# yusuke1127/RoboManipBaselines

Measured on AMD Instinct MI355X. Metric: env-steps/s (whole node) + policy-inference us/step, MujocoUR5eCable x N ACT, higher is better.
Workload: dtype f64 physics + fp32 policy; 1 GPU; MujocoUR5eCable x1024 (1024 per GPU), ACT (ResNet-18 + transformer 4/7 layers, chunk 100, skip 3, temporal ensembling), fp32 policy, RolloutPhase hot loop; num_envs_per_gpu=1024, total_envs=1024, parallelism=single GPU (no collective), env_groups=1, act_decoder_layers_run=1

## Files before the change

include/rmbx.h:

```cpp
#ifndef RMBX_H_
#define RMBX_H_

#include <stddef.h>
#include <stdint.h>

#ifdef __cplusplus
extern "C" {
#endif

#define RMBX_OK 0
#define RMBX_ERR_ARG -1
#define RMBX_ERR_HIP -2
#define RMBX_ERR_STATE -3

#define RMBX_ABI_VERSION 2

int rmbx_abi_version(void);
const char* rmbx_last_error(void);
int rmbx_device_count(int* count);

int rmbx_act_ensemble(const float* new_chunk, const uint8_t* push, const uint8_t* active,
                      float* hist, int32_t* hist_len, int32_t* hist_head,
                      const double* w_table, const double* dn_scale, const double* dn_sub,
                      const double* dn_add, double* out, int n_env, int chunk, int adim,
// ... 228 lines not shown
int rmbx_conv3x3_f16x3_patch(const float* in, int N, int H, int W, int C, const void* w_planes,
                             long long w_plane_stride, const float* w_scale, const float* bias, const float* res,
                             float* out, int Cout, int relu, void* stream);
int rmbx_conv2d_f16x3(const float* in, int N, int H, int W, int C, const void* w_planes, const float* w_scale,
                      const float* bias, const float* res, float* out, int Cout, int KH, int KW, int stride, int pad,
                      int relu, void* stream);
int rmbx_attention_f32x6(const float* q, const float* k, const float* v, float* out, int B, int heads, int Lq, int Lk,
                         long long q_bstride, int q_rstride, long long k_bstride, int k_rstride, long long v_bstride,
                         int v_rstride, float scale, void* stream);
int rmbx_attention_f16x3(const float* q, const float* k, const float* v, float* out, int* redo, int B, int heads,
                         int Lq, int Lk, long long q_bstride, int q_rstride, long long k_bstride, int k_rstride,
                         long long v_bstride, int v_rstride, float scale, void* stream);
int rmbx_groupnorm_act(const float* x, const float* weight, const float* bias, float* out, int B, int C, int T,
                       int groups, float eps, int mish, void* stream);
int rmbx_add_layernorm(const void* x, const void* r, const float* weight, const float* bias, void* out,
                       int rows, int D, float eps, int dtype, void* stream);
int rmbx_add_layernorm_pos(const void* x, const void* r, const float* weight, const float* bias, void* out,
                           const void* pos, int pos_rows, void* out_pos, int rows, int D, float eps, int dtype,
                           void* stream);
int rmbx_add_layernorm_split(const float* x, const float* r, const float* weight, const float* bias, float* out,
                             void* y_planes, float* y_rinv, float* y_norm, const float* pos, int pos_rows,
                             float* out_pos, void* pos_planes, float* pos_rinv, int rows, int D, float eps,
                             void* stream);
int rmbx_nhwc_bias_relu_maxpool(const void* x, const float* bias, void* out, int N, int H, int W,
                                int C, int dtype, void* stream);

int rmbx_ddpm_step(const float* model_output, const float* sample, const float* noise,
                   float* prev_sample, size_t n, const float* coeffs, void* stream);
int rmbx_ddim_step(const float* model_output, const float* sample, float* prev_sample, size_t n,
                   const float* coeffs, int eps_mode, void* stream);

int rmbx_resize_crop_u8(const uint8_t* src, int n_env, int H, int W, int C, int rh, int rw, int y0,
                        int x0, int ch, int cw, float a, float b, void* dst, int dst_dtype,
                        void* stream);
int rmbx_resize_f32(const float* src, float* dst, int n_env, int H, int W, int rh, int rw,
                    void* stream);

int rmbx_pointcloud_fps(const float* depth, const uint8_t* rgb, int n_env, int H, int W,
                        double focal_scaling, const double* min_bound, const double* max_bound,
                        int K, int norm_type, const double* norm_a, const double* norm_b,
                        const double* norm_c, float* out, double* raw, int32_t* count,
                        void* stream);

#ifdef __cplusplus
}
#endif
// ... 3 lines not shown
```

robomanipbaselines_amd/_native.py:

```python

import ctypes
import os

import numpy as np

_LIB_PATH = os.path.join(os.path.dirname(os.path.abspath(__file__)), "_lib",
                         f"librmbx_{os.environ['RMBX_LIB_VARIANT']}.so" if os.environ.get("RMBX_LIB_VARIANT")
                         else "librmbx.so")

_c_int = ctypes.c_int
_c_p = ctypes.c_void_p
_c_sz = ctypes.c_size_t
_c_d = ctypes.c_double

SIGNATURES = {
    "rmbx_abi_version": (_c_int, []),
    "rmbx_last_error": (ctypes.c_char_p, []),
    "rmbx_device_count": (_c_int, [_c_p]),
    "rmbx_act_ensemble": (
        _c_int,
        [_c_p] * 11 + [_c_int, _c_int, _c_int, _c_int, _c_p],
    ),
    "rmbx_cable_reward": (_c_int, [_c_p] * 5 + [_c_int, _c_int, _c_p]),
    "rmbx_door_reward": (_c_int, [_c_p, _c_p, _c_p, _c_p, _c_int, _c_d, _c_d, _c_p]),
# ... 42 lines not shown
    "rmbx_attention_f16x3": (_c_int, [_c_p] * 5 + [_c_int] * 4 + [ctypes.c_longlong, _c_int] * 3 + [ctypes.c_float, _c_p]),
    "rmbx_linear_f32x6": (_c_int, [_c_p, ctypes.c_longlong, _c_p, ctypes.c_longlong, ctypes.c_longlong, _c_p, _c_p,
                                   ctypes.c_longlong, _c_int, _c_int, _c_int, _c_int, _c_p]),
    "rmbx_conv2d_f32x6": (_c_int, [_c_p] + [_c_int] * 4 + [_c_p] * 4 + [_c_int] * 6 + [_c_p]),
    "rmbx_linear_f32x6_batched": (_c_int, [_c_p, ctypes.c_longlong, ctypes.c_longlong, _c_p, ctypes.c_longlong,
                                           ctypes.c_longlong, ctypes.c_longlong, _c_p, _c_p, ctypes.c_longlong,
                                           ctypes.c_longlong] + [_c_int] * 5 + [_c_p]),
    "rmbx_wino4_input_f32": (_c_int, [_c_p] + [_c_int] * 4 + [_c_p, _c_p]),
    "rmbx_wino4_output_f32": (_c_int, [_c_p] + [_c_int] * 4 + [_c_p] * 3 + [_c_int, _c_p]),
    "rmbx_conv2d_direct_f32": (_c_int, [_c_p] + [_c_int] * 4 + [_c_p] * 3 + [_c_int] * 5 + [_c_p]),
    "rmbx_split_bf16x3": (_c_int, [_c_p, _c_p, ctypes.c_longlong, _c_p]),
    "rmbx_split_f16x2": (_c_int, [_c_p, _c_int, _c_int, _c_p, _c_p, _c_p]),
    "rmbx_linear_f16x3": (_c_int, [_c_p, ctypes.c_longlong, _c_p, ctypes.c_longlong, ctypes.c_longlong, _c_p, _c_p,
                                   _c_p, ctypes.c_longlong, _c_int, _c_int, _c_int, _c_int, _c_p]),
    "rmbx_linear_f16x3_batched": (_c_int, [_c_p, ctypes.c_longlong, ctypes.c_longlong, _c_p, ctypes.c_longlong,
                                           ctypes.c_longlong, ctypes.c_longlong, _c_p, ctypes.c_longlong, _c_p, _c_p,
                                           ctypes.c_longlong, ctypes.c_longlong] + [_c_int] * 5 + [_c_p]),
    "rmbx_conv3x3_f16x3_patch": (_c_int, [_c_p] + [_c_int] * 4 + [_c_p, ctypes.c_longlong] + [_c_p] * 4
                                 + [_c_int, _c_int, _c_p]),
    "rmbx_conv2d_f16x3": (_c_int, [_c_p] + [_c_int] * 4 + [_c_p] * 5 + [_c_int] * 6 + [_c_p]),
    "rmbx_add_layernorm": (_c_int, [_c_p] * 5 + [_c_int, _c_int, ctypes.c_float, _c_int, _c_p]),
    "rmbx_groupnorm_act": (_c_int, [_c_p] * 4 + [_c_int] * 4 + [ctypes.c_float, _c_int, _c_p]),
    "rmbx_add_layernorm_split": (_c_int, [_c_p] * 9 + [_c_int, _c_p, _c_p, _c_p, _c_int, _c_int, ctypes.c_float, _c_p]),
    "rmbx_linear_f16x3_presplit_split": (_c_int, [_c_p, ctypes.c_longlong, ctypes.c_longlong, _c_p, _c_p, _c_p,
                                                  ctypes.c_longlong, ctypes.c_longlong, _c_p, ctypes.c_float,
                                                  ctypes.c_float, _c_p, _c_int, _c_p, ctypes.c_longlong,
                                                  ctypes.c_longlong, _c_p, _c_int, _c_int, _c_int, _c_p]),
    "rmbx_linear_f16x3_presplit_batched": (_c_int, [_c_p, ctypes.c_longlong, ctypes.c_longlong, ctypes.c_longlong, _c_p,
                                                    ctypes.c_longlong, _c_p, ctypes.c_longlong, ctypes.c_longlong,
                                                    ctypes.c_longlong, _c_p, ctypes.c_longlong, _c_p, _c_p,
                                                    ctypes.c_longlong, ctypes.c_longlong, _c_int, _c_int, _c_int, _c_int,
                                                    _c_int, _c_p]),
    "rmbx_wino4_input_split": (_c_int, [_c_p, _c_int, _c_int, _c_int, _c_int, _c_p, _c_p, _c_p]),
    "rmbx_linear_f16x3_presplit": (_c_int, [_c_p, ctypes.c_longlong, ctypes.c_longlong, _c_p, _c_p, ctypes.c_longlong,
                                            ctypes.c_longlong, _c_p, _c_p, _c_p, _c_p, ctypes.c_longlong, _c_int, _c_int,
                                            _c_int, _c_int, _c_p]),
    "rmbx_add_layernorm_pos": (_c_int, [_c_p] * 6 + [_c_int, _c_p, _c_int, _c_int, ctypes.c_float, _c_int, _c_p]),
    "rmbx_ddpm_step": (_c_int, [_c_p] * 4 + [_c_sz, _c_p, _c_p]),
    "rmbx_ddim_step": (_c_int, [_c_p] * 3 + [_c_sz, _c_p, _c_int, _c_p]),
    "rmbx_resize_crop_u8": (_c_int, [_c_p] + [_c_int] * 10 + [ctypes.c_float, ctypes.c_float, _c_p, _c_int, _c_p]),
    "rmbx_resize_f32": (_c_int, [_c_p, _c_p] + [_c_int] * 5 + [_c_p]),
    "rmbx_pointcloud_fps": (_c_int, [_c_p, _c_p, _c_int, _c_int, _c_int, _c_d, _c_p, _c_p, _c_int, _c_int,
                                     _c_p, _c_p, _c_p, _c_p, _c_p, _c_p, _c_p]),
}


# ... 99 lines not shown
```

robomanipbaselines_amd/csrc/rmbx_nn.hip:

```cpp

#include "rmbx_common.h"

#include <cstdint>
#include <type_traits>

namespace rmbx {
namespace {

__device__ __forceinline__ float bf2f(uint16_t h) { return __uint_as_float((uint32_t)h << 16); }

__device__ __forceinline__ uint16_t f2bf(float f) {
  uint32_t u = __float_as_uint(f);
  if ((u & 0x7fffffffu) > 0x7f800000u) return 0x7fc0;
  u += 0x7fffu + ((u >> 16) & 1u);
  return (uint16_t)(u >> 16);
}

struct BF16 {
  static constexpr int VEC = 8;
  using vec_t = uint4;
  __device__ static void unpack(const vec_t& v, float* f) {
    const uint32_t w[4] = {v.x, v.y, v.z, v.w};
#pragma unroll
    for (int i = 0; i < 4; ++i) {
// ... 164 lines not shown
  const int g = rmbx::grid_for((size_t)N * Ho * Wo * cvec);
  if (dtype == 1)
    hipLaunchKernelGGL(rmbx::bias_relu_maxpool_kernel<rmbx::BF16>, dim3(g), dim3(256), 0, s,
                       (const uint4*)x, bias, (uint4*)out, N, H, W, cvec, Ho, Wo);
  else
    hipLaunchKernelGGL(rmbx::bias_relu_maxpool_kernel<rmbx::F32>, dim3(g), dim3(256), 0, s,
                       (const float4*)x, bias, (float4*)out, N, H, W, cvec, Ho, Wo);
  RMBX_CHECK_LAUNCH();
  return RMBX_OK;
}

namespace rmbx {
namespace {

struct LnSplit {
  uint16_t* y_planes;
  float* y_rinv;
  uint16_t* pos_planes;
  float* pos_rinv;
  int rows;
  float* y_norm;
};

template <class T, int PER>
__global__ void __launch_bounds__(256) add_layernorm_kernel(const typename T::vec_t* __restrict__ x,
                                                            const typename T::vec_t* __restrict__ r,
                                                            const float* __restrict__ w, const float* __restrict__ b,
                                                            typename T::vec_t* __restrict__ out, int rows, int D,
                                                            float eps, const typename T::vec_t* __restrict__ pos,
                                                            int pos_rows, typename T::vec_t* __restrict__ out_pos,
                                                            LnSplit sp) {
  constexpr int V = T::VEC;
  const int lane = threadIdx.x & 63;
  const int row = blockIdx.x * 4 + (threadIdx.x >> 6);
  if (row >= rows) return;
  const int nvec = D / V;
  const size_t base = (size_t)row * nvec;
  float s[PER][V], s2[PER][V];
  float sum = 0.f;
#pragma unroll
  for (int q = 0; q < PER; ++q) {
    const int v = lane + q * 64;
    if (v < nvec) {
      float a[V], c[V];
      T::unpack(x[base + v], a);
      if (r) {
        T::unpack(r[base + v], c);
#pragma unroll
        for (int k = 0; k < V; ++k) a[k] = T::round(a[k] + c[k]);
      }
#pragma unroll
      for (int k = 0; k < V; ++k) {
        s[q][k] = a[k];
        sum += a[k];
      }
    } else {
#pragma unroll
      for (int k = 0; k < V; ++k) s[q][k] = 0.f;
    }
  }
#pragma unroll
  for (int off = 32; off > 0; off >>= 1) sum += __shfl_xor(sum, off);
  const float mean = sum / (float)D;
  float var = 0.f;
#pragma unroll
  for (int q = 0; q < PER; ++q) {
    const int v = lane + q * 64;
    if (v < nvec) {
#pragma unroll
      for (int k = 0; k < V; ++k) {
// ... 34 lines not shown
#pragma unroll
        for (int k = 0; k < V; ++k) yr[k] = yr[k] + pv[k];
        const typename T::vec_t pvv = T::pack(yr);
        if (out_pos) out_pos[base + v] = pvv;
        if (sp.pos_planes) {
          T::unpack(pvv, yr);
#pragma unroll
          for (int k = 0; k < V; ++k) pmax = fmaxf(pmax, fabsf(yr[k]));
        }
      }
      {
        float t[V];
        T::unpack(yv, t);
#pragma unroll
        for (int k = 0; k < V; ++k) s[q][k] = t[k];
      }
      if (sp.pos_planes) {
#pragma unroll
        for (int k = 0; k < V; ++k) s2[q][k] = yr[k];
      }
    }
  }
  if constexpr (std::is_same<T, F32>::value) {
    auto split_row = [&](float (*vals)[V], float mx, uint16_t* planes, float* rinv) {
#pragma unroll
      for (int off = 32; off > 0; off >>= 1) mx = fmaxf(mx, __shfl_xor(mx, off));
      int e = 14;
      if (mx > 0.f && mx <= 3.4e38f) frexpf(mx, &e);
      const float sc = ldexpf(1.f, 14 - e);
      if (lane == 0) rinv[row] = ldexpf(1.f, e - 14);
      const size_t plane = (size_t)sp.rows * D;
#pragma unroll
      for (int q = 0; q < PER; ++q) {
        const int v = lane + q * 64;
        if (v < nvec) {
          uint16_t h[V], l[V];
#pragma unroll
          for (int k = 0; k < V; ++k) {
            const float a = vals[q][k] * sc;
            const _Float16 hv = (_Float16)a;
            h[k] = __builtin_bit_cast(uint16_t, hv);
            l[k] = __builtin_bit_cast(uint16_t, (_Float16)(a - (float)hv));
          }
          static_assert(V == 4, "f32 rows move as float4");
          const size_t o = (size_t)row * D + (size_t)v * V;
          *(uint2*)(planes + o) = make_uint2(h[0] | ((uint32_t)h[1] << 16), h[2] | ((uint32_t)h[3] << 16));
          *(uint2*)(planes + plane + o) = make_uint2(l[0] | ((uint32_t)l[1] << 16), l[2] | ((uint32_t)l[3] << 16));
        }
      }
    };
    if (sp.y_norm) {
      float q = ysq;
#pragma unroll
      for (int off = 32; off > 0; off >>= 1) q += __shfl_xor(q, off);
      if (lane == 0) sp.y_norm[row] = sqrtf(q) * (1.f + 0.000244140625f);
    }
    if (sp.y_planes) split_row(s, ymax, sp.y_planes, sp.y_rinv);
    if (sp.pos_planes) split_row(s2, pmax, sp.pos_planes, sp.pos_rinv);
  }
}

}
}

extern "C" int rmbx_add_layernorm_pos(const void* x, const void* r, const float* weight, const float* bias, void* out,
                                      const void* pos, int pos_rows, void* out_pos, int rows, int D, float eps,
                                      int dtype, void* stream);

extern "C" int rmbx_add_layernorm(const void* x, const void* r, const float* weight, const float* bias, void* out,
                                  int rows, int D, float eps, int dtype, void* stream) {
  return rmbx_add_layernorm_pos(x, r, weight, bias, out, nullptr, 0, nullptr, rows, D, eps, dtype, stream);
}

namespace {
int add_layernorm_impl(const void* x, const void* r, const float* weight, const float* bias, void* out,
                       const void* pos, int pos_rows, void* out_pos, int rows, int D, float eps, int dtype,
                       void* stream, rmbx::LnSplit sp) {
  RMBX_CHECK_ARG(!(out_pos || sp.pos_planes) || (pos && pos_rows > 0),
                 "rmbx_add_layernorm_pos: out_pos needs pos and pos_rows > 0");
  RMBX_CHECK_ARG(((uintptr_t)pos | (uintptr_t)out_pos) % 16 == 0, "rmbx_add_layernorm_pos: unaligned");
  RMBX_CHECK_ARG(x && weight && bias && (out || sp.y_planes || sp.pos_planes), "rmbx_add_layernorm: null pointer");
  RMBX_CHECK_ARG(dtype == 0 || dtype == 1, "rmbx_add_layernorm: dtype must be 0 (f32) or 1 (bf16)");
  const int vec = dtype == 1 ? 8 : 4;
  RMBX_CHECK_ARG(D > 0 && D % vec == 0 && D <= 2048, "rmbx_add_layernorm: D=%d must be a multiple of %d, <= 2048",
                 D, vec);
  RMBX_CHECK_ARG(((uintptr_t)x | (uintptr_t)r | (uintptr_t)out) % 16 == 0, "rmbx_add_layernorm: unaligned");
  if (rows <= 0) return RMBX_OK;
  hipStream_t s = (hipStream_t)stream;
  const int grid = (rows + 3) / 4;
  const int nvec = D / vec;
  if (dtype == 1) {
    if (nvec <= 64)
      hipLaunchKernelGGL((rmbx::add_layernorm_kernel<rmbx::BF16, 1>), dim3(grid), dim3(256), 0, s, (const uint4*)x,
                         (const uint4*)r, weight, bias, (uint4*)out, rows, D, eps, (const uint4*)pos, pos_rows,
                         (uint4*)out_pos, sp);
    else if (nvec <= 128)
      hipLaunchKernelGGL((rmbx::add_layernorm_kernel<rmbx::BF16, 2>), dim3(grid), dim3(256), 0, s, (const uint4*)x,
                         (const uint4*)r, weight, bias, (uint4*)out, rows, D, eps, (const uint4*)pos, pos_rows,
                         (uint4*)out_pos, sp);
    else
      hipLaunchKernelGGL((rmbx::add_layernorm_kernel<rmbx::BF16, 4>), dim3(grid), dim3(256), 0, s, (const uint4*)x,
                         (const uint4*)r, weight, bias, (uint4*)out, rows, D, eps, (const uint4*)pos, pos_rows,
                         (uint4*)out_pos, sp);
  } else {
    if (nvec <= 64)
      hipLaunchKernelGGL((rmbx::add_layernorm_kernel<rmbx::F32, 1>), dim3(grid), dim3(256), 0, s, (const float4*)x,
                         (const float4*)r, weight, bias, (float4*)out, rows, D, eps, (const float4*)pos, pos_rows,
                         (float4*)out_pos, sp);
    else if (nvec <= 128)
      hipLaunchKernelGGL((rmbx::add_layernorm_kernel<rmbx::F32, 2>), dim3(grid), dim3(256), 0, s, (const float4*)x,
                         (const float4*)r, weight, bias, (float4*)out, rows, D, eps, (const float4*)pos, pos_rows,
                         (float4*)out_pos, sp);
    else if (nvec <= 256)
      hipLaunchKernelGGL((rmbx::add_layernorm_kernel<rmbx::F32, 4>), dim3(grid), dim3(256), 0, s, (const float4*)x,
                         (const float4*)r, weight, bias, (float4*)out, rows, D, eps, (const float4*)pos, pos_rows,
                         (float4*)out_pos, sp);
    else
      hipLaunchKernelGGL((rmbx::add_layernorm_kernel<rmbx::F32, 8>), dim3(grid), dim3(256), 0, s, (const float4*)x,
                         (const float4*)r, weight, bias, (float4*)out, rows, D, eps, (const float4*)pos, pos_rows,
                         (float4*)out_pos, sp);
  }
  RMBX_CHECK_LAUNCH();
  return RMBX_OK;
}
}

extern "C" int rmbx_add_layernorm_pos(const void* x, const void* r, const float* weight, const float* bias, void* out,
                                      const void* pos, int pos_rows, void* out_pos, int rows, int D, float eps,
                                      int dtype, void* stream) {
  return add_layernorm_impl(x, r, weight, bias, out, pos, pos_rows, out_pos, rows, D, eps, dtype, stream,
                            rmbx::LnSplit{nullptr, nullptr, nullptr, nullptr, rows, nullptr});
}

extern "C" int rmbx_add_layernorm_split(const float* x, const float* r, const float* weight, const float* bias,
                                        float* out, void* y_planes, float* y_rinv, float* y_norm, const float* pos,
                                        int pos_rows, float* out_pos, void* pos_planes, float* pos_rinv, int rows, int D,
                                        float eps, void* stream) {
  RMBX_CHECK_ARG(!y_planes == !y_rinv && !pos_planes == !pos_rinv, "rmbx_add_layernorm_split: planes need their rinv");
  RMBX_CHECK_ARG(D % 4 == 0 && ((uintptr_t)y_planes | (uintptr_t)pos_planes) % 8 == 0,
                 "rmbx_add_layernorm_split: D %% 4 and 8-byte aligned planes");
  return add_layernorm_impl(x, r, weight, bias, out, pos, pos_rows, out_pos, rows, D, eps, 0, stream,
                            rmbx::LnSplit{(uint16_t*)y_planes, y_rinv, (uint16_t*)pos_planes, pos_rinv, rows, y_norm});
}

namespace rmbx {
namespace {

__device__ __forceinline__ float gn_block_sum(float v, float* red) {
#pragma unroll
  for (int o = 32; o > 0; o >>= 1) v += __shfl_xor(v, o);
  const int wave = threadIdx.x >> 6;
  __syncthreads();
  if ((threadIdx.x & 63) == 0) red[wave] = v;
  __syncthreads();
  return red[0] + red[1] + red[2] + red[3];
}

constexpr int GN_REG = 8;
template <bool MISH, bool TIN>
__global__ void __launch_bounds__(256) groupnorm_act_kernel(const float* __restrict__ x, const float* __restrict__ w,
                                                            const float* __restrict__ b, float* __restrict__ y, int C,
                                                            int T, int G, float eps) {
  __shared__ float red[4];
  const int bg = blockIdx.x, g = bg % G, cg = C / G;
  const int E = cg * T, tid = threadIdx.x;
// ... 93 lines not shown
```

robomanipbaselines_amd/kernels.py:

```python

import os
import numpy as np
import torch

from . import _native as N


def _chk(t, dtype, shape=None, name="tensor"):
    if not isinstance(t, torch.Tensor):
        raise ValueError(f"{name} must be a torch.Tensor")
    if not t.is_cuda:
        raise ValueError(f"{name} must be a device tensor (got {t.device})")
    if t.dtype != dtype:
        raise ValueError(f"{name} must be {dtype} (got {t.dtype})")
    if not t.is_contiguous():
        raise ValueError(f"{name} must be contiguous")
    if shape is not None and tuple(t.shape) != tuple(shape):
        raise ValueError(f"{name} must have shape {tuple(shape)} (got {tuple(t.shape)})")
    return t


def ensemble_weight_table(chunk, k=0.01):
    w = np.zeros((chunk, chunk), dtype=np.float64)
    for n in range(1, chunk + 1):
# ... 477 lines not shown
                      torch.empty(rows, dtype=torch.float32, device=x.device) if y_norm else None) if split_y else None
    yp = ps = pos2 = None
    if pos is not None:
        pos2 = pos.reshape(-1, D)
        if pos2.dtype != x.dtype or not pos2.is_contiguous() or not pos2.is_cuda:
            raise ValueError("pos must be a contiguous device tensor of x's dtype")
        if x.dim() < 2 or x.shape[-2] % pos2.shape[0] != 0:
            raise ValueError("pos rows must divide the sequence length")
        yp = torch.empty_like(x)
        if split_pos:
            ps = PresplitRows(torch.empty((2, rows, D), dtype=torch.float16, device=x.device),
                              torch.empty(rows, dtype=torch.float32, device=x.device))
    N.call("rmbx_add_layernorm_split", N.ptr(x), N.ptr(r), N.ptr(weight), N.ptr(bias), N.ptr(y),
           N.ptr(ys.planes if ys else None), N.ptr(ys.rinv if ys else None), N.ptr(ys.norm if ys else None), N.ptr(pos2),
           pos2.shape[0] if pos2 is not None else 0, N.ptr(yp), N.ptr(ps.planes if ps else None),
           N.ptr(ps.rinv if ps else None), rows, D, float(eps), N.stream_ptr())
    if ys is not None:
        ys.bind(y)
        y.rmbx_split = ys
    if ps is not None:
        ps.bind(yp)
        yp.rmbx_split = ps
    return (y, yp) if pos is not None else y


def weight_bounds(w, b):
    wn = float(w.detach().double().norm(dim=1).max()) if w.numel() else 0.0
    bm = float(b.detach().double().abs().max()) if b is not None and b.numel() else 0.0
    up = 1.0 + 2.0 ** -20
    return wn * up, bm * up


def linear_presplit_split(xs, planes, bias, bounds, relu=False, out=None):
    Nn, K, h3 = _planes_nk(planes, "linear_presplit_split")
    if not h3 or xs.norm is None or xs.planes.shape[2] != K:
        raise ValueError("linear_presplit_split: f16x3 planes and pre-split rows with norm bounds of width K")
    M = xs.planes.shape[1]
    if bias is not None:
        _chk(bias, torch.float32, (Nn,), "bias")
    if out is None:
        out = PresplitRows(torch.empty((2, M, Nn), dtype=torch.float16, device=xs.planes.device),
                           torch.empty(M, dtype=torch.float32, device=xs.planes.device))
    elif (tuple(out.planes.shape) != (2, M, Nn) or out.planes.dtype != torch.float16 or out.planes.stride(2) != 1
          or tuple(out.rinv.shape) != (M,) or out.rinv.dtype != torch.float32 or not out.rinv.is_contiguous()):
        raise ValueError("linear_presplit_split: out must hold [2, M, N] f16 planes (unit column stride) and [M] f32 rinv")
    p, ap, op = planes.planes, xs.planes, out.planes
# ... 606 lines not shown
```

robomanipbaselines_amd/policy/act/act_model.py:

```python

import math
import os

import torch
import torch.nn as nn
import torch.nn.functional as F

from ..backbone import FusedResNet18Trunk, ResNet18Trunk

IMAGENET_MEAN = (0.485, 0.456, 0.406)
IMAGENET_STD = (0.229, 0.224, 0.225)


def sine_pos_embed(h, w, num_pos_feats=256, temperature=10000, device=None, dtype=torch.float32):
    scale = 2 * math.pi
    eps = 1e-6
    ones = torch.ones(1, h, w, device=device, dtype=torch.float32)
    y_embed = ones.cumsum(1)
    x_embed = ones.cumsum(2)
    y_embed = y_embed / (y_embed[:, -1:, :] + eps) * scale
    x_embed = x_embed / (x_embed[:, :, -1:] + eps) * scale
    dim_t = torch.arange(num_pos_feats, dtype=torch.float32, device=device)
    dim_t = temperature ** (2 * (dim_t // 2) / num_pos_feats)
    pos_x = x_embed[:, :, :, None] / dim_t
# ... 81 lines not shown
    def _out_proj(self, o):
        if self.fused_attention and _x6_ok(o, self.out_proj.out_features):
            return _x6_linear(self, "out_proj", o, self.out_proj.weight, self.out_proj.bias)
        return self.out_proj(o)

    def forward(self, q, k, v):
        D = q.shape[2]
        if q is k and k is v:
            qkv = self._in_proj(q, 0, 3 * D)
            qq, kk, vv = qkv.split(D, dim=-1)
        elif q is k:
            qk = self._in_proj(q, 0, 2 * D)
            qq, kk = qk.split(D, dim=-1)
            vv = self._in_proj(v, 2 * D, 3 * D)
        else:
            qq = self._in_proj(q, 0, D)
            kk = self._in_proj(k, D, 2 * D)
            vv = self._in_proj(v, 2 * D, 3 * D)
        return self._attend(qq, kk, vv)

    def attend_kv(self, q, kk, vv):
        D = q.shape[2]
        return self._attend(self._in_proj(q, 0, D), kk, vv)

    def _attend(self, qq, kk, vv):
        B, Lq, D = qq.shape
        Lk = kk.shape[1]
        hd = D // self.h
        if self.fused_attention and qq.dtype == torch.bfloat16 and hd == 64 and Lk <= 320 and qq.is_cuda:
            from ... import kernels as K

            return self._out_proj(K.attention_bf16(qq, kk, vv, self.h))
        if self.fused_attention and qq.dtype == torch.float32 and hd == 64 and qq.is_cuda:
            from ... import kernels as K

            return self._out_proj(K.attention_f32(qq, kk, vv, self.h, form=F32_ATTN))
        qq = qq.view(B, Lq, self.h, hd).transpose(1, 2)
        kk = kk.view(B, Lk, self.h, hd).transpose(1, 2)
        vv = vv.view(B, Lk, self.h, hd).transpose(1, 2)
        o = F.scaled_dot_product_attention(qq, kk, vv)
        return self.out_proj(o.transpose(1, 2).reshape(B, Lq, D))


class _LayerOps(nn.Module):

    fused = False
# ... 28 lines not shown
        cache = norm.__dict__.get("_f32")
        if cache is None or cache[0] != key:
            cache = (key, norm.weight.detach().float().contiguous(), norm.bias.detach().float().contiguous())
            norm.__dict__["_f32"] = cache
        return cache[1], cache[2]

    @staticmethod
    def _presplit(x):
        from ... import kernels as K

        return (x.dtype == torch.float32 and F32_GEMM == "x6" and K.F32_PIECES == "f16x3" and K.GEMM_PRESPLIT
                and x.is_cuda and x.shape[-1] % K.LINEAR_F32X6_BK == 0)

    def addnorm(self, norm, x, r):
        if self.fused:
            from ... import kernels as K

            w, b = self._norm_f32(norm)
            if self._presplit(x):
                return K.add_layernorm_split(x.contiguous(), r.contiguous(), w, b, norm.eps, y_norm=True)
            return K.add_layernorm(x.contiguous(), r.contiguous(), w, b, norm.eps)
        return norm(x + r)

    def addnorm_pos(self, norm, x, r, pos):
        if self.fused:
            from ... import kernels as K

            w, b = self._norm_f32(norm)
            if self._presplit(x):
                return K.add_layernorm_split(x.contiguous(), r.contiguous(), w, b, norm.eps, pos=pos.contiguous(),
                                             split_y=False)
            return K.add_layernorm_pos(x.contiguous(), r.contiguous(), w, b, pos.contiguous(), norm.eps)
        y = norm(x + r)
        return y, y + pos


class EncoderLayer(_LayerOps):
    def __init__(self, d, heads, ff):
        super().__init__()
        self.self_attn = MHA(d, heads)
        self.linear1, self.linear2 = nn.Linear(d, ff), nn.Linear(ff, d)
        self.norm1, self.norm2 = nn.LayerNorm(d), nn.LayerNorm(d)

    def forward(self, src, pos):
        q = src + pos
        src = self.addnorm(self.norm1, src, self.self_attn(q, q, src))
        return self.addnorm(self.norm2, src, self.ffn(src))

    def forward_q(self, src, q, pos, want_next_q):
        src = self.addnorm(self.norm1, src, self.self_attn(q, q, src))
        if want_next_q:
            return self.addnorm_pos(self.norm2, src, self.ffn(src), pos)
        return self.addnorm(self.norm2, src, self.ffn(src)), None


class DecoderLayer(_LayerOps):
    def __init__(self, d, heads, ff):
        super().__init__()
        self.self_attn = MHA(d, heads)
        self.multihead_attn = MHA(d, heads)
        self.linear1, self.linear2 = nn.Linear(d, ff), nn.Linear(ff, d)
        self.norm1, self.norm2, self.norm3 = nn.LayerNorm(d), nn.LayerNorm(d), nn.LayerNorm(d)

    def forward(self, tgt, memory, pos, query_pos, mem_pos=None):
        q = tgt + query_pos
        tgt = self.addnorm(self.norm1, tgt, self.self_attn(q, q, tgt))
        mk = memory + pos if mem_pos is None else mem_pos
        tgt = self.addnorm(self.norm2, tgt, self.multihead_attn(tgt + query_pos, mk, memory))
        return self.addnorm(self.norm3, tgt, self.ffn(tgt))

    def forward_q(self, tgt, q, memory, query_pos, mem_pos, want_next_q, cross_kv=None):
        tgt, q2 = self.addnorm_pos(self.norm1, tgt, self.self_attn(q, q, tgt), query_pos)
        if cross_kv is not None:
            ca = self.multihead_attn.attend_kv(q2, *cross_kv)
        else:
            ca = self.multihead_attn(q2, mem_pos, memory)
        tgt = self.addnorm(self.norm2, tgt, ca)
        if want_next_q:
            return self.addnorm_pos(self.norm3, tgt, self.ffn(tgt), query_pos)
        return self.addnorm(self.norm3, tgt, self.ffn(tgt)), None


class ActModel(nn.Module):

    def __init__(self, state_dim=7, action_dim=7, num_queries=100, hidden_dim=512, dim_feedforward=3200,
                 nheads=8, enc_layers=4, dec_layers=7, num_cams=1, latent_dim=32):
        super().__init__()
        d = hidden_dim
        self.num_queries, self.num_cams, self.latent_dim = num_queries, num_cams, latent_dim
        self.backbone = ResNet18Trunk()
        self.input_proj = nn.Conv2d(512, d, kernel_size=1)
        self.input_proj_robot_state = nn.Linear(state_dim, d)
        self.latent_out_proj = nn.Linear(latent_dim, d)
        self.query_embed = nn.Embedding(num_queries, d)
        self.additional_pos_embed = nn.Embedding(2, d)
        self.encoder_layers = nn.ModuleList([EncoderLayer(d, nheads, dim_feedforward) for _ in range(enc_layers)])
        self.decoder_layers = nn.ModuleList([DecoderLayer(d, nheads, dim_feedforward) for _ in range(dec_layers)])
        self.decoder_norm = nn.LayerNorm(d)
        self.action_head = nn.Linear(d, action_dim)
        self.is_pad_head = nn.Linear(d, 1)
# ... 20 lines not shown
        layers = self.decoder_layers[:n_dec]
        if not self.batch_cross_kv or n_dec < 2 or not all(getattr(l, "fused", False) for l in layers):
            return None
        D = mem.shape[2]
        ws = [l.multihead_attn.in_proj_weight for l in layers]
        bs = [l.multihead_attn.in_proj_bias for l in layers]
        key = tuple((w.data_ptr(), w.dtype) for w in ws)
        cache = self.__dict__.get("_cross_w")
        if cache is None or cache[0] != key:
            wk = torch.cat([w[D: 2 * D] for w in ws]).contiguous()
            bk = torch.cat([b[D: 2 * D] for b in bs]).contiguous()
            wv = torch.cat([w[2 * D:] for w in ws]).contiguous()
            bv = torch.cat([b[2 * D:] for b in bs]).contiguous()
            cache = (key, wk, bk, wv, bv)
            self.__dict__["_cross_w"] = cache
        _, wk, bk, wv, bv = cache
        if _x6_ok(mem, wk.shape[0]):
            k_all = _x6_linear(self, "cross_k", mem_pos, wk, bk)
            v_all = _x6_linear(self, "cross_v", mem, wv, bv)
        else:
            k_all = F.linear(mem_pos, wk, bk)
            v_all = F.linear(mem, wv, bv)
        return [(k_all[..., i * D: (i + 1) * D], v_all[..., i * D: (i + 1) * D]) for i in range(n_dec)]

    def _input_proj(self, feat):
        c = self.input_proj
        if (self._fused is not None and feat.is_contiguous(memory_format=torch.channels_last)
                and _x6_ok(feat.permute(0, 2, 3, 1), c.out_channels)):
            y = _x6_linear(self, "input_proj", feat.permute(0, 2, 3, 1), c.weight.view(c.out_channels, -1), c.bias)
            return y.permute(0, 3, 1, 2)
        return c(feat)

    def _pos(self, h, w, device, dtype):
        key = (h, w, str(device), dtype)
        if key not in self._pos_cache:
            self._pos_cache[key] = sine_pos_embed(h, w, self.input_proj.out_channels // 2, device=device, dtype=dtype)
        return self._pos_cache[key]

    @property
    def accepts_s2d(self):
        return self._fused is not None

    @property
    def accepts_u8_s2d(self):
        return (self._fused is not None and self._fused.stem.conv.weight.dtype == torch.float32
                and os.environ.get("RMBX_STEM_U8", "1") != "0")
# ... 6 lines not shown
            raise ValueError("ActModel: 8-bit images must be the space-to-depth form of the fused device model")
        feats, poss = [], []
        for c in range(image.shape[1]):
            x = image[:, c]
            if image.dtype == torch.uint8:
                f = self._input_proj(trunk.forward_s2d_u8(x.contiguous(), *self.u8_image_norm))
            elif s2d:
                f = self._input_proj(trunk.forward_s2d(x.contiguous()))
            else:
                if self._fused is not None:
                    x = x.contiguous(memory_format=torch.channels_last)
                f = self._input_proj(trunk(x))
            feats.append(f)
            poss.append(self._pos(f.shape[2], f.shape[3], f.device, f.dtype))
        src = (feats[0] if len(feats) == 1 else torch.cat(feats, dim=3)).flatten(2).transpose(1, 2)
        pos = (poss[0] if len(poss) == 1 else torch.cat(poss, dim=3)).flatten(2).transpose(1, 2)
        dev_f32 = self._fused is not None and src.is_cuda and src.dtype == torch.float32 and F32_GEMM == "x6"
        latent = self.latent_out_proj(torch.zeros(B, self.latent_dim, device=qpos.device, dtype=src.dtype))
        if dev_f32:
            p = self.input_proj_robot_state
            proprio = _x6_linear_padded(self, "proprio", qpos.to(src.dtype).contiguous(), p.weight, p.bias)
        else:
            proprio = self.input_proj_robot_state(qpos.to(src.dtype))
        src = torch.cat([latent[:, None], proprio[:, None], src], dim=1)
        pos = torch.cat([self.additional_pos_embed.weight[None].to(src.dtype), pos], dim=1)
        mem = src
        q = src + pos
        n_enc = len(self.encoder_layers)
        for i, layer in enumerate(self.encoder_layers):
            mem, q = layer.forward_q(mem, q, pos, want_next_q=True)
        qe = self.query_embed.weight[None].to(src.dtype)
        tgt = torch.zeros(B, self.num_queries, mem.shape[2], device=mem.device, dtype=mem.dtype)
        mem_pos = q if q is not None else mem + pos
        q = tgt + qe
        first = None
        n_dec = 1 if self.prune_dead_decoder else len(self.decoder_layers)
        cross = self._cross_kv(mem_pos, mem, n_dec)
        for i in range(n_dec):
            tgt, q = self.decoder_layers[i].forward_q(tgt, q, mem, qe, mem_pos, want_next_q=i + 1 < n_dec,
                                                      cross_kv=cross[i] if cross else None)
            if i == 0:
                if dev_f32:
                    from ... import kernels as K

                    w, b = _LayerOps._norm_f32(self.decoder_norm)
                    first = K.add_layernorm(tgt.contiguous(), None, w, b, self.decoder_norm.eps)
                else:
                    first = self.decoder_norm(tgt)
        if dev_f32:
            h = self.action_head
            return _x6_linear_padded(self, "action_head", first.contiguous(), h.weight, h.bias)
        return self.action_head(first)


def normalize_images(image):
    m = torch.tensor(IMAGENET_MEAN, device=image.device, dtype=image.dtype).reshape(1, 1, 3, 1, 1)
    s = torch.tensor(IMAGENET_STD, device=image.device, dtype=image.dtype).reshape(1, 1, 3, 1, 1)
    return (image - m) / s
```

Before: 22520 env-steps/s.

## Fold batch-independent decoder prefix and fuse encoder input concat with pre-split

The first decoder layer's self-attention, norm1 and cross-attention query projection act on zero targets plus learned query embeddings, so they are the same for every environment. They are now computed once for batch 1, cached under a key built from weight pointers and versions, and broadcast through a new add-layernorm kernel that indexes the residual with a row modulus. Separately, the encoder input concat, the positional add and the fp16 hi/lo pre-split of q are merged into one kernel, so the first encoder layer's QK projection consumes pre-split planes. This cuts per-step decoder GEMM/attention work and several elementwise passes, at the cost of cache-invalidation complexity and extra code paths.

```diff
diff --git a/include/rmbx.h b/include/rmbx.h
--- a/include/rmbx.h
+++ b/include/rmbx.h
@@ -274,6 +274,11 @@
                              void* y_planes, float* y_rinv, float* y_norm, const float* pos, int pos_rows,
                              float* out_pos, void* pos_planes, float* pos_rinv, int rows, int D, float eps,
                              void* stream);
+int rmbx_add_layernorm_bcast(const void* x, const void* r, int r_rows, const float* weight, const float* bias,
+                             void* out, void* y_planes, float* y_rinv, float* y_norm, int rows, int D, float eps,
+                             int dtype, void* stream);
+int rmbx_encoder_input_split(const float* proj, const float* head0, const float* head1, const float* pos, float* src,
+                             void* planes, float* rinv, int B, int L, int D, void* stream);
 int rmbx_nhwc_bias_relu_maxpool(const void* x, const float* bias, void* out, int N, int H, int W,
                                 int C, int dtype, void* stream);
 
diff --git a/robomanipbaselines_amd/_native.py b/robomanipbaselines_amd/_native.py
--- a/robomanipbaselines_amd/_native.py
+++ b/robomanipbaselines_amd/_native.py
@@ -88,6 +88,8 @@
     "rmbx_add_layernorm": (_c_int, [_c_p] * 5 + [_c_int, _c_int, ctypes.c_float, _c_int, _c_p]),
     "rmbx_groupnorm_act": (_c_int, [_c_p] * 4 + [_c_int] * 4 + [ctypes.c_float, _c_int, _c_p]),
     "rmbx_add_layernorm_split": (_c_int, [_c_p] * 9 + [_c_int, _c_p, _c_p, _c_p, _c_int, _c_int, ctypes.c_float, _c_p]),
+    "rmbx_add_layernorm_bcast": (_c_int, [_c_p, _c_p, _c_int] + [_c_p] * 6 + [_c_int, _c_int, ctypes.c_float, _c_int, _c_p]),
+    "rmbx_encoder_input_split": (_c_int, [_c_p] * 7 + [_c_int] * 3 + [_c_p]),
     "rmbx_linear_f16x3_presplit_split": (_c_int, [_c_p, ctypes.c_longlong, ctypes.c_longlong, _c_p, _c_p, _c_p,
                                                   ctypes.c_longlong, ctypes.c_longlong, _c_p, ctypes.c_float,
                                                   ctypes.c_float, _c_p, _c_int, _c_p, ctypes.c_longlong,
diff --git a/robomanipbaselines_amd/csrc/rmbx_nn.hip b/robomanipbaselines_amd/csrc/rmbx_nn.hip
--- a/robomanipbaselines_amd/csrc/rmbx_nn.hip
+++ b/robomanipbaselines_amd/csrc/rmbx_nn.hip
@@ -210,6 +210,37 @@
   float* y_norm;
 };
 
+template <int PER>
+__device__ __forceinline__ void split_row_f32(float (*vals)[4], float mx, uint16_t* planes, float* rinv, int row,
+                                              int lane, int D, int rows) {
+  constexpr int V = 4;
+  const int nvec = D / V;
+#pragma unroll
+  for (int off = 32; off > 0; off >>= 1) mx = fmaxf(mx, __shfl_xor(mx, off));
+  int e = 14;
+  if (mx > 0.f && mx <= 3.4e38f) frexpf(mx, &e);
+  const float sc = ldexpf(1.f, 14 - e);
+  if (lane == 0) rinv[row] = ldexpf(1.f, e - 14);
+  const size_t plane = (size_t)rows * D;
+#pragma unroll
+  for (int q = 0; q < PER; ++q) {
+    const int v = lane + q * 64;
+    if (v < nvec) {
+      uint16_t h[V], l[V];
+#pragma unroll
+      for (int k = 0; k < V; ++k) {
+        const float a = vals[q][k] * sc;
+        const _Float16 hv = (_Float16)a;
+        h[k] = __builtin_bit_cast(uint16_t, hv);
+        l[k] = __builtin_bit_cast(uint16_t, (_Float16)(a - (float)hv));
+      }
+      const size_t o = (size_t)row * D + (size_t)v * V;
+      *(uint2*)(planes + o) = make_uint2(h[0] | ((uint32_t)h[1] << 16), h[2] | ((uint32_t)h[3] << 16));
+      *(uint2*)(planes + plane + o) = make_uint2(l[0] | ((uint32_t)l[1] << 16), l[2] | ((uint32_t)l[3] << 16));
+    }
+  }
+}
+
 template <class T, int PER>
 __global__ void __launch_bounds__(256) add_layernorm_kernel(const typename T::vec_t* __restrict__ x,
                                                             const typename T::vec_t* __restrict__ r,
@@ -217,13 +248,14 @@
                                                             typename T::vec_t* __restrict__ out, int rows, int D,
                                                             float eps, const typename T::vec_t* __restrict__ pos,
                                                             int pos_rows, typename T::vec_t* __restrict__ out_pos,
-                                                            LnSplit sp) {
+                                                            LnSplit sp, int r_rows) {
   constexpr int V = T::VEC;
   const int lane = threadIdx.x & 63;
   const int row = blockIdx.x * 4 + (threadIdx.x >> 6);
   if (row >= rows) return;
   const int nvec = D / V;
   const size_t base = (size_t)row * nvec;
+  const size_t rbase = r_rows > 0 ? (size_t)(row % r_rows) * nvec : base;
   float s[PER][V], s2[PER][V];
   float sum = 0.f;
 #pragma unroll
@@ -233,7 +265,7 @@
       float a[V], c[V];
       T::unpack(x[base + v], a);
       if (r) {
-        T::unpack(r[base + v], c);
+        T::unpack(r[rbase + v], c);
 #pragma unroll
         for (int k = 0; k < V; ++k) a[k] = T::round(a[k] + c[k]);
       }
@@ -314,42 +346,51 @@
     }
   }
   if constexpr (std::is_same<T, F32>::value) {
-    auto split_row = [&](float (*vals)[V], float mx, uint16_t* planes, float* rinv) {
-#pragma unroll
-      for (int off = 32; off > 0; off >>= 1) mx = fmaxf(mx, __shfl_xor(mx, off));
-      int e = 14;
-      if (mx > 0.f && mx <= 3.4e38f) frexpf(mx, &e);
-      const float sc = ldexpf(1.f, 14 - e);
-      if (lane == 0) rinv[row] = ldexpf(1.f, e - 14);
-      const size_t plane = (size_t)sp.rows * D;
-#pragma unroll
-      for (int q = 0; q < PER; ++q) {
-        const int v = lane + q * 64;
-        if (v < nvec) {
-          uint16_t h[V], l[V];
-#pragma unroll
-          for (int k = 0; k < V; ++k) {
-            const float a = vals[q][k] * sc;
-            const _Float16 hv = (_Float16)a;
-            h[k] = __builtin_bit_cast(uint16_t, hv);
-            l[k] = __builtin_bit_cast(uint16_t, (_Float16)(a - (float)hv));
-          }
-          static_assert(V == 4, "f32 rows move as float4");
-          const size_t o = (size_t)row * D + (size_t)v * V;
-          *(uint2*)(planes + o) = make_uint2(h[0] | ((uint32_t)h[1] << 16), h[2] | ((uint32_t)h[3] << 16));
-          *(uint2*)(planes + plane + o) = make_uint2(l[0] | ((uint32_t)l[1] << 16), l[2] | ((uint32_t)l[3] << 16));
-        }
-      }
-    };
     if (sp.y_norm) {
       float q = ysq;
 #pragma unroll
       for (int off = 32; off > 0; off >>= 1) q += __shfl_xor(q, off);
       if (lane == 0) sp.y_norm[row] = sqrtf(q) * (1.f + 0.000244140625f);
     }
-    if (sp.y_planes) split_row(s, ymax, sp.y_planes, sp.y_rinv);
-    if (sp.pos_planes) split_row(s2, pmax, sp.pos_planes, sp.pos_rinv);
-  }
+    if (sp.y_planes) split_row_f32<PER>(s, ymax, sp.y_planes, sp.y_rinv, row, lane, D, sp.rows);
+    if (sp.pos_planes) split_row_f32<PER>(s2, pmax, sp.pos_planes, sp.pos_rinv, row, lane, D, sp.rows);
+  }
+}
+
+template <int PER>
+__global__ void __launch_bounds__(256) encoder_input_kernel(const float4* __restrict__ proj,
+                                                            const float4* __restrict__ head0,
+                                                            const float4* __restrict__ head1,
+                                                            const float4* __restrict__ pos, float4* __restrict__ src,
+                                                            uint16_t* __restrict__ planes, float* __restrict__ rinv,
+                                                            int B, int L, int D) {
+  const int lane = threadIdx.x & 63;
+  const int rows = B * (L + 2);
+  const int row = blockIdx.x * 4 + (threadIdx.x >> 6);
+  if (row >= rows) return;
+  const int nvec = D / 4;
+  const int b = row / (L + 2), t = row - b * (L + 2);
+  const float4* in = t == 0   ? head0 + (size_t)b * nvec
+                     : t == 1 ? head1 + (size_t)b * nvec
+                              : proj + ((size_t)b * L + (t - 2)) * nvec;
+  float s[PER][4];
+  float mx = 0.f;
+#pragma unroll
+  for (int q = 0; q < PER; ++q) {
+    const int v = lane + q * 64;
+    if (v < nvec) {
+      const float4 a = in[v];
+      src[(size_t)row * nvec + v] = a;
+      const float4 p = pos[(size_t)t * nvec + v];
+      s[q][0] = a.x + p.x;
+      s[q][1] = a.y + p.y;
+      s[q][2] = a.z + p.z;
+      s[q][3] = a.w + p.w;
+#pragma unroll
+      for (int k = 0; k < 4; ++k) mx = fmaxf(mx, fabsf(s[q][k]));
+    }
+  }
+  split_row_f32<PER>(s, mx, planes, rinv, row, lane, D, rows);
 }
 
 }
@@ -367,7 +408,7 @@
 namespace {
 int add_layernorm_impl(const void* x, const void* r, const float* weight, const float* bias, void* out,
                        const void* pos, int pos_rows, void* out_pos, int rows, int D, float eps, int dtype,
-                       void* stream, rmbx::LnSplit sp) {
+                       void* stream, rmbx::LnSplit sp, int r_rows = 0) {
   RMBX_CHECK_ARG(!(out_pos || sp.pos_planes) || (pos && pos_rows > 0),
                  "rmbx_add_layernorm_pos: out_pos needs pos and pos_rows > 0");
   RMBX_CHECK_ARG(((uintptr_t)pos | (uintptr_t)out_pos) % 16 == 0, "rmbx_add_layernorm_pos: unaligned");
@@ -385,32 +426,32 @@
     if (nvec <= 64)
       hipLaunchKernelGGL((rmbx::add_layernorm_kernel<rmbx::BF16, 1>), dim3(grid), dim3(256), 0, s, (const uint4*)x,
                          (const uint4*)r, weight, bias, (uint4*)out, rows, D, eps, (const uint4*)pos, pos_rows,
-                         (uint4*)out_pos, sp);
+                         (uint4*)out_pos, sp, r_rows);
     else if (nvec <= 128)
       hipLaunchKernelGGL((rmbx::add_layernorm_kernel<rmbx::BF16, 2>), dim3(grid), dim3(256), 0, s, (const uint4*)x,
                          (const uint4*)r, weight, bias, (uint4*)out, rows, D, eps, (const uint4*)pos, pos_rows,
-                         (uint4*)out_pos, sp);
+                         (uint4*)out_pos, sp, r_rows);
     else
       hipLaunchKernelGGL((rmbx::add_layernorm_kernel<rmbx::BF16, 4>), dim3(grid), dim3(256), 0, s, (const uint4*)x,
                          (const uint4*)r, weight, bias, (uint4*)out, rows, D, eps, (const uint4*)pos, pos_rows,
-                         (uint4*)out_pos, sp);
+                         (uint4*)out_pos, sp, r_rows);
   } else {
     if (nvec <= 64)
       hipLaunchKernelGGL((rmbx::add_layernorm_kernel<rmbx::F32, 1>), dim3(grid), dim3(256), 0, s, (const float4*)x,
                          (const float4*)r, weight, bias, (float4*)out, rows, D, eps, (const float4*)pos, pos_rows,
-                         (float4*)out_pos, sp);
+                         (float4*)out_pos, sp, r_rows);
     else if (nvec <= 128)
       hipLaunchKernelGGL((rmbx::add_layernorm_kernel<rmbx::F32, 2>), dim3(grid), dim3(256), 0, s, (const float4*)x,
                          (const float4*)r, weight, bias, (float4*)out, rows, D, eps, (const float4*)pos, pos_rows,
-                         (float4*)out_pos, sp);
+                         (float4*)out_pos, sp, r_rows);
     else if (nvec <= 256)
       hipLaunchKernelGGL((rmbx::add_layernorm_kernel<rmbx::F32, 4>), dim3(grid), dim3(256), 0, s, (const float4*)x,
                          (const float4*)r, weight, bias, (float4*)out, rows, D, eps, (const float4*)pos, pos_rows,
-                         (float4*)out_pos, sp);
+                         (float4*)out_pos, sp, r_rows);
     else
       hipLaunchKernelGGL((rmbx::add_layernorm_kernel<rmbx::F32, 8>), dim3(grid), dim3(256), 0, s, (const float4*)x,
                          (const float4*)r, weight, bias, (float4*)out, rows, D, eps, (const float4*)pos, pos_rows,
-                         (float4*)out_pos, sp);
+                         (float4*)out_pos, sp, r_rows);
   }
   RMBX_CHECK_LAUNCH();
   return RMBX_OK;
@@ -433,6 +474,43 @@
                  "rmbx_add_layernorm_split: D %% 4 and 8-byte aligned planes");
   return add_layernorm_impl(x, r, weight, bias, out, pos, pos_rows, out_pos, rows, D, eps, 0, stream,
                             rmbx::LnSplit{(uint16_t*)y_planes, y_rinv, (uint16_t*)pos_planes, pos_rinv, rows, y_norm});
+}
+
+extern "C" int rmbx_add_layernorm_bcast(const void* x, const void* r, int r_rows, const float* weight,
+                                        const float* bias, void* out, void* y_planes, float* y_rinv, float* y_norm,
+                                        int rows, int D, float eps, int dtype, void* stream) {
+  RMBX_CHECK_ARG(r && r_rows > 0, "rmbx_add_layernorm_bcast: r and r_rows > 0 are required");
+  RMBX_CHECK_ARG(!y_planes == !y_rinv, "rmbx_add_layernorm_bcast: planes need their rinv");
+  RMBX_CHECK_ARG(dtype == 0 || !(y_planes || y_norm), "rmbx_add_layernorm_bcast: the pre-split outputs are f32 only");
+  RMBX_CHECK_ARG(D % 4 == 0 && (uintptr_t)y_planes % 8 == 0, "rmbx_add_layernorm_bcast: D %% 4 and 8-byte aligned planes");
+  return add_layernorm_impl(x, r, weight, bias, out, nullptr, 0, nullptr, rows, D, eps, dtype, stream,
+                            rmbx::LnSplit{(uint16_t*)y_planes, y_rinv, nullptr, nullptr, rows, y_norm}, r_rows);
+}
+
+extern "C" int rmbx_encoder_input_split(const float* proj, const float* head0, const float* head1, const float* pos,
+                                        float* src, void* planes, float* rinv, int B, int L, int D, void* stream) {
+  RMBX_CHECK_ARG(proj && head0 && head1 && pos && src && planes && rinv, "rmbx_encoder_input_split: null pointer");
+  RMBX_CHECK_ARG(B >= 0 && L >= 0 && (long long)B * (L + 2) < (1ll << 31) - 4,
+                 "rmbx_encoder_input_split: B=%d, L=%d out of range", B, L);
+  RMBX_CHECK_ARG(D > 0 && D % 4 == 0 && D <= 2048, "rmbx_encoder_input_split: D=%d must be a multiple of 4, <= 2048", D);
+  RMBX_CHECK_ARG(((uintptr_t)proj | (uintptr_t)head0 | (uintptr_t)head1 | (uintptr_t)pos | (uintptr_t)src) % 16 == 0 &&
+                     (uintptr_t)planes % 8 == 0,
+                 "rmbx_encoder_input_split: unaligned");
+  if (B == 0) return RMBX_OK;
+  hipStream_t s = (hipStream_t)stream;
+  const int grid = (B * (L + 2) + 3) / 4;
+  const int nvec = D / 4;
+#define RMBX_EI(PER)                                                                                              \
+  hipLaunchKernelGGL(rmbx::encoder_input_kernel<PER>, dim3(grid), dim3(256), 0, s, (const float4*)proj,           \
+                     (const float4*)head0, (const float4*)head1, (const float4*)pos, (float4*)src, (uint16_t*)planes, \
+                     rinv, B, L, D)
+  if (nvec <= 64) RMBX_EI(1);
+  else if (nvec <= 128) RMBX_EI(2);
+  else if (nvec <= 256) RMBX_EI(4);
+  else RMBX_EI(8);
+#undef RMBX_EI
+  RMBX_CHECK_LAUNCH();
+  return RMBX_OK;
 }
 
 namespace rmbx {
diff --git a/robomanipbaselines_amd/kernels.py b/robomanipbaselines_amd/kernels.py
--- a/robomanipbaselines_amd/kernels.py
+++ b/robomanipbaselines_amd/kernels.py
@@ -523,6 +523,52 @@
         ps.bind(yp)
         yp.rmbx_split = ps
     return (y, yp) if pos is not None else y
+
+
+def add_layernorm_bcast(x, r, weight, bias, eps=1e-5, split=False, y_norm=False):
+    if x.dtype not in _NN_DTYPES or not x.is_cuda or not x.is_contiguous():
+        raise ValueError("x must be a contiguous bf16/f32 device tensor")
+    D = x.shape[-1]
+    r2 = r.reshape(-1, D)
+    if r2.dtype != x.dtype or not r2.is_contiguous() or r2.device != x.device:
+        raise ValueError("r must be a contiguous tensor of x's dtype on x's device")
+    if x.dim() < 2 or x.shape[-2] % r2.shape[0] != 0:
+        raise ValueError("r rows must divide the sequence length")
+    if split and x.dtype != torch.float32:
+        raise ValueError("the pre-split form is f32 only")
+    _chk(weight, torch.float32, (D,), "weight")
+    _chk(bias, torch.float32, (D,), "bias")
+    rows = x.numel() // D
+    y = torch.empty_like(x)
+    ys = PresplitRows(torch.empty((2, rows, D), dtype=torch.float16, device=x.device),
+                      torch.empty(rows, dtype=torch.float32, device=x.device),
+                      torch.empty(rows, dtype=torch.float32, device=x.device) if y_norm else None) if split else None
+    N.call("rmbx_add_layernorm_bcast", N.ptr(x), N.ptr(r2), r2.shape[0], N.ptr(weight), N.ptr(bias), N.ptr(y),
+           N.ptr(ys.planes if ys else None), N.ptr(ys.rinv if ys else None), N.ptr(ys.norm if ys else None), rows, D,
+           float(eps), _NN_DTYPES[x.dtype], N.stream_ptr())
+    if ys is not None:
+        ys.bind(y)
+        y.rmbx_split = ys
+    return y
+
+
+def encoder_input_split(proj, head0, head1, pos):
+    _chk(proj, torch.float32, name="proj")
+    if proj.dim() != 3 or not proj.is_cuda:
+        raise ValueError("proj must be an f32 [B, L, D] device tensor")
+    B, L, D = proj.shape
+    pos2 = pos.reshape(-1, D)
+    for t, shp, nm in ((head0, (B, D), "head0"), (head1, (B, D), "head1"), (pos2, (L + 2, D), "pos")):
+        _chk(t, torch.float32, shp, nm)
+        if t.device != proj.device:
+            raise ValueError(f"{nm} must be on {proj.device} (got {t.device})")
+    rows = B * (L + 2)
+    src = torch.empty((B, L + 2, D), dtype=torch.float32, device=proj.device)
+    qs = PresplitRows(torch.empty((2, rows, D), dtype=torch.float16, device=proj.device),
+                      torch.empty(rows, dtype=torch.float32, device=proj.device))
+    N.call("rmbx_encoder_input_split", N.ptr(proj), N.ptr(head0), N.ptr(head1), N.ptr(pos2), N.ptr(src),
+           N.ptr(qs.planes), N.ptr(qs.rinv), B, L, D, N.stream_ptr())
+    return src, qs
 
 
 def weight_bounds(w, b):
diff --git a/robomanipbaselines_amd/policy/act/act_model.py b/robomanipbaselines_amd/policy/act/act_model.py
--- a/robomanipbaselines_amd/policy/act/act_model.py
+++ b/robomanipbaselines_amd/policy/act/act_model.py
@@ -127,6 +127,24 @@
     def attend_kv(self, q, kk, vv):
         D = q.shape[2]
         return self._attend(self._in_proj(q, 0, D), kk, vv)
+
+    def forward_presplit_qk(self, qs, v):
+        from ... import kernels as K
+
+        B, L, D = v.shape
+        w, bb = self.in_proj_weight, self.in_proj_bias
+        qk = K.linear_presplit(qs, _x6_planes(self, "in_proj", w)[:, 0: 2 * D], bb[0: 2 * D]).view(B, L, 2 * D)
+        qq, kk = qk.split(D, dim=-1)
+        return self._attend(qq, kk, self._in_proj(v, 2 * D, 3 * D))
+
+    def attend_qproj(self, qq, k, v, cross_kv=None):
+        D = qq.shape[2]
+        if cross_kv is not None:
+            kk, vv = cross_kv
+        else:
+            kk = self._in_proj(k, D, 2 * D)
+            vv = self._in_proj(v, 2 * D, 3 * D)
+        return self._attend(qq.expand(kk.shape[0], -1, -1), kk, vv)
 
     def _attend(self, qq, kk, vv):
         B, Lq, D = qq.shape
@@ -201,6 +219,15 @@
             return K.add_layernorm(x.contiguous(), r.contiguous(), w, b, norm.eps)
         return norm(x + r)
 
+    def addnorm_bcast(self, norm, x1, r):
+        if self.fused:
+            from ... import kernels as K
+
+            w, b = self._norm_f32(norm)
+            split = self._presplit(r)
+            return K.add_layernorm_bcast(r.contiguous(), x1.contiguous(), w, b, norm.eps, split=split, y_norm=split)
+        return norm(x1 + r)
+
     def addnorm_pos(self, norm, x, r, pos):
         if self.fused:
             from ... import kernels as K
@@ -227,7 +254,11 @@
         return self.addnorm(self.norm2, src, self.ffn(src))
 
     def forward_q(self, src, q, pos, want_next_q):
-        src = self.addnorm(self.norm1, src, self.self_attn(q, q, src))
+        if isinstance(q, torch.Tensor):
+            sa = self.self_attn(q, q, src)
+        else:
+            sa = self.self_attn.forward_presplit_qk(q, src)
+        src = self.addnorm(self.norm1, src, sa)
         if want_next_q:
             return self.addnorm_pos(self.norm2, src, self.ffn(src), pos)
         return self.addnorm(self.norm2, src, self.ffn(src)), None
@@ -255,6 +286,13 @@
         else:
             ca = self.multihead_attn(q2, mem_pos, memory)
         tgt = self.addnorm(self.norm2, tgt, ca)
+        if want_next_q:
+            return self.addnorm_pos(self.norm3, tgt, self.ffn(tgt), query_pos)
+        return self.addnorm(self.norm3, tgt, self.ffn(tgt)), None
+
+    def forward_folded(self, tgt1, qq, memory, query_pos, mem_pos, want_next_q, cross_kv=None):
+        ca = self.multihead_attn.attend_qproj(qq, mem_pos, memory, cross_kv)
+        tgt = self.addnorm_bcast(self.norm2, tgt1, ca)
         if want_next_q:
             return self.addnorm_pos(self.norm3, tgt, self.ffn(tgt), query_pos)
         return self.addnorm(self.norm3, tgt, self.ffn(tgt)), None
@@ -321,6 +359,36 @@
             k_all = F.linear(mem_pos, wk, bk)
             v_all = F.linear(mem, wv, bv)
         return [(k_all[..., i * D: (i + 1) * D], v_all[..., i * D: (i + 1) * D]) for i in range(n_dec)]
+
+    fold_decoder_prefix = True
+
+    def _decoder_prefix(self, device, dtype):
+        if not self.fold_decoder_prefix or len(self.decoder_layers) == 0:
+            return None
+        l0 = self.decoder_layers[0]
+        sa, ca = l0.self_attn, l0.multihead_attn
+        if not (l0.fused and sa.fused_attention and ca.fused_attention) or torch.device(device).type != "cuda":
+            return None
+        qe = self.query_embed.weight[None].to(dtype)
+        D = qe.shape[2]
+        if not (_x6_ok(qe, D) and _x6_ok(qe, 2 * D)):
+            return None
+        ts = (self.query_embed.weight, sa.in_proj_weight, sa.in_proj_bias, sa.out_proj.weight, sa.out_proj.bias,
+              l0.norm1.weight, l0.norm1.bias, ca.in_proj_weight, ca.in_proj_bias)
+        from ... import kernels as K
+
+        modes = (F32_GEMM, F32_ATTN, K.F32_PIECES, K.GEMM_PRESPLIT)
+        key = (str(device), dtype, l0.norm1.eps, modes) + tuple((t.data_ptr(), t._version, t.dtype) for t in ts)
+        cache = self.__dict__.get("_dec_prefix")
+        if cache is None or cache[0] != key:
+            with torch.no_grad():
+                tgt = torch.zeros(1, self.num_queries, D, device=device, dtype=dtype)
+                q = tgt + qe
+                tgt1, q2 = l0.addnorm_pos(l0.norm1, tgt, sa(q, q, tgt), qe)
+                qq = ca._in_proj(q2, 0, D)
+            cache = (key, tgt1, qq)
+            self.__dict__["_dec_prefix"] = cache
+        return cache[1], cache[2]
 
     def _input_proj(self, feat):
         c = self.input_proj
@@ -373,23 +441,37 @@
             proprio = _x6_linear_padded(self, "proprio", qpos.to(src.dtype).contiguous(), p.weight, p.bias)
         else:
             proprio = self.input_proj_robot_state(qpos.to(src.dtype))
-        src = torch.cat([latent[:, None], proprio[:, None], src], dim=1)
         pos = torch.cat([self.additional_pos_embed.weight[None].to(src.dtype), pos], dim=1)
+        l0 = self.encoder_layers[0] if len(self.encoder_layers) else None
+        if (dev_f32 and l0 is not None and l0.fused and l0.self_attn.fused_attention and _LayerOps._presplit(src)
+                and _x6_ok(src, 2 * src.shape[2]) and (2 * src.shape[2]) % 128 == 0):
+            from ... import kernels as K
+
+            src, q = K.encoder_input_split(src.contiguous(), latent.contiguous(), proprio.contiguous(),
+                                           pos.contiguous())
+        else:
+            src = torch.cat([latent[:, None], proprio[:, None], src], dim=1)
+            q = src + pos
         mem = src
-        q = src + pos
         n_enc = len(self.encoder_layers)
         for i, layer in enumerate(self.encoder_layers):
             mem, q = layer.forward_q(mem, q, pos, want_next_q=True)
         qe = self.query_embed.weight[None].to(src.dtype)
-        tgt = torch.zeros(B, self.num_queries, mem.shape[2], device=mem.device, dtype=mem.dtype)
         mem_pos = q if q is not None else mem + pos
-        q = tgt + qe
         first = None
         n_dec = 1 if self.prune_dead_decoder else len(self.decoder_layers)
         cross = self._cross_kv(mem_pos, mem, n_dec)
+        prefix = self._decoder_prefix(mem.device, mem.dtype) if n_dec > 0 else None
+        if prefix is None:
+            tgt = torch.zeros(B, self.num_queries, mem.shape[2], device=mem.device, dtype=mem.dtype)
+            q = tgt + qe
         for i in range(n_dec):
-            tgt, q = self.decoder_layers[i].forward_q(tgt, q, mem, qe, mem_pos, want_next_q=i + 1 < n_dec,
-                                                      cross_kv=cross[i] if cross else None)
+            if i == 0 and prefix is not None:
+                tgt, q = self.decoder_layers[0].forward_folded(*prefix, mem, qe, mem_pos, want_next_q=n_dec > 1,
+                                                               cross_kv=cross[0] if cross else None)
+            else:
+                tgt, q = self.decoder_layers[i].forward_q(tgt, q, mem, qe, mem_pos, want_next_q=i + 1 < n_dec,
+                                                          cross_kv=cross[i] if cross else None)
             if i == 0:
                 if dev_f32:
                     from ... import kernels as K
```

Measured after the change: 22870 env-steps/s, median of 6. 1.02x the previous value.
